# belinghy/SteppingStone

Measured on AMD Instinct MI355X. Metric: env-steps/sec (batched random-action rollout), higher is better.
Workload: dtype f32; 1 GPU; Walker3DStepperEnv-v0, 4096 envs per MI355X, curriculum 0 (flat terrain), on-device Philox U(-1,1) actions, auto-reset on; envs_total=4096, parallelism=env-shard x1, ranks=1, steps_per_launch=1000, prewarm_steps=256

## Files before the change

steppingstone_amd/csrc/ss_dynamics.hpp:

```cpp
#pragma once
#include "ss_math.hpp"
#include "ss_pair.hpp"

namespace ss {

constexpr float kH = 1.0f / 240.0f;
constexpr float kDt = 1.0f / 60.0f;
constexpr float kGrav = 9.8f;
constexpr float kPlankA = kStonePlankHalfLength, kPlankB = kStonePlankHalfWidth;
constexpr int kPgsIters = 5;
constexpr float kErp = 0.2f;
constexpr float kSlop = 0.001f;
constexpr float kVcorrMax = 2.0f;


constexpr int kWave = 64;
constexpr int kEnvsPerWave = 32;
constexpr int kLdsSlots = 40;
constexpr int kSlotsA = 20;
constexpr int kLdsC = 0;
constexpr int kLdsT = 18;
constexpr int kLdsHead = 36;
constexpr int kScalarBase = kSlotsA * kWave * 4;
constexpr int kRecWords = 9;
constexpr int kCholWords = 15 + 6;
constexpr int kHandJc = 0, kHandL0 = kHandJc + 8 * kRecWords, kHandLc = kHandL0 + kCholWords, kHandDet = 129, kHandAct = 146, kHandFloats = 158, kHandCs = kHandLc;
constexpr bool bias_offload(int helpers) { return helpers >= 3; }
constexpr bool spine_packed(int helpers) { return helpers >= 3; }
constexpr bool torques_paired(int helpers, bool kstep) { return helpers >= 3 && kstep; }
constexpr bool response_from_lds(int helpers, bool kstep) { return helpers >= 3 && kstep; }
constexpr int kHandBias = kHandJc;
static_assert(24 <= 3 * kRecWords, "biases fit the spine records' place");
constexpr int kHandRows = kHandJc + 3 * kRecWords;
constexpr int kHandRows3 = 160;
constexpr int kHandFloats3 = kHandRows3 + 40;
constexpr int kHandSlots3 = (kHandFloats3 + 3) / 4;
constexpr int hand_slots(int helpers) { return helpers >= 3 ? kHandSlots3 : (kHandFloats + 3) / 4; }
constexpr bool rows_offload(int helpers) { return helpers >= 3; }
constexpr int kHandSlots = (kHandFloats + 3) / 4;
static_assert(kLdsSlots + kHandSlots <= 80, "two helper-variant workgroups must fit the 160 KiB of a CU (16384 envs: 512 workgroups)");
static_assert(kHandRows + 40 <= kHandJc + 8 * kRecWords, "rows fit the leg records' place");
constexpr int kHandBase = kLdsSlots * kWave * 4;
constexpr int kFarWord0 = kHandLc;
constexpr int kFarBytes = (kHandBase + kFarWord0 * kWave) * 4;
static_assert(kFarBytes <= 65536, "every hand-off word beyond the offset field of the lane's own base goes through the far base");
constexpr bool hand_far(int idx) { return idx >= kFarWord0; }
constexpr int hand_far_offset(int idx) { return (idx - kFarWord0) * kWave * 4; }
constexpr int lds_bytes(int helpers) { return (kLdsSlots + hand_slots(helpers)) * kWave * 16; }
constexpr int hand_last_word(int helpers) { return hand_slots(helpers) * 4 - 1; }
static_assert(kHandFloats3 - 1 <= hand_last_word(3) && kHandFloats + 2 - 1 <= hand_last_word(1), "the words in use (one helper: + kHandOut2's two) are allocated");
static_assert(kFarBytes + (kWave - 1) * 4 + hand_far_offset(hand_last_word(1)) + 4 <= lds_bytes(1), "one helper: far base + largest word is inside the allocation");
static_assert(kFarBytes + (kWave - 1) * 4 + hand_far_offset(hand_last_word(3)) + 4 <= lds_bytes(3), "three helpers: far base + largest word is inside the allocation");
static_assert(hand_far_offset(kFarWord0) == 0 && hand_far_offset(hand_last_word(3)) < 65536 && hand_far_offset(hand_last_word(1)) < 65536,
              "every far offset fits the 16-bit offset field");
static_assert(hand_far_offset(1) - hand_far_offset(0) == 256 && hand_far_offset(hand_last_word(3)) / 256 <= 255,
              "far offsets are multiples of 256 B within ds_*2st64_b32's reach");
constexpr int NH = 12;
enum { S_ACT = 0, S_Q = 12, S_QD = 24, S_WLAM = 36, S_POS = 48, S_QUAT = 51, S_VW = 55, S_VV = 58, S_STP = 61, S_STN = 70,
       S_WKEY = 79, S_END = 80 };
static_assert(S_END <= (kLdsSlots - kSlotsA) * 4, "LDS scalar region overflow");
constexpr bool warm_in_lds(int helpers) { return helpers < 3; }

constexpr int kHalf[NH] = {0, 1, 2, 3, 4, 5, 6, 7, 13, 14, 15, 16};
constexpr int left_twin(int jr) { return jr < 3 ? jr : (jr < 8 ? jr + 5 : jr + 4); }
constexpr bool mirror_flips(int j) { return kAxis[j] != 1; }
__host__ __device__ constexpr float mirror_sign(int j, float m) { return mirror_flips(j) ? m : 1.f; }
__host__ __device__ constexpr float action_lane_sign(int jr, float m) {
  return jr < 3 ? mirror_sign(jr, m) : (float)kPolicySign[jr];
}
__host__ __device__ constexpr float policy_true_sign(int jr, int side) {
  return jr < 3 ? 1.f : (float)kPolicySign[jr] * ((mirror_flips(jr) && side) ? -1.f : 1.f);
}
constexpr int first_child_half(int b) {
  int r = -1;
  for (int i = 0; i < NH; ++i)
    if (kParent[kHalf[i]] == b) r = kHalf[i] + 1;
  return r;
}

#define SS_MEMBAR() asm volatile("" ::: "memory")
#if defined(__HIP_DEVICE_COMPILE__)
#define SS_WAVE_SYNC() asm volatile("" ::: "memory")
#else
#define SS_WAVE_SYNC() ss_host_wave_sync()
#endif

#if defined(SS_PROFILE_PHASES) && defined(__HIP_DEVICE_COMPILE__)
struct Prof { uint32_t t[16]; uint32_t last; };
#define SS_PROF_DECL Prof& prof,
#define SS_PROF_ARG prof,
#define SS_PROF_RAW(i) do { uint32_t _n = __builtin_amdgcn_readfirstlane((uint32_t)__builtin_amdgcn_s_memtime()); \
    prof.t[i] = __builtin_amdgcn_readfirstlane(prof.t[i] + (_n - __builtin_amdgcn_readfirstlane(prof.last))); prof.last = _n; } while (0)
#ifdef SS_PROFILE_EPILOGUE
#define SS_PROF(i) SS_PROF_RAW(0)
#define SS_PROFE(i) SS_PROF_RAW(i)
#else
#define SS_PROF(i) SS_PROF_RAW(i)
#define SS_PROFE(i) ((void)0)
#endif
#else
#define SS_PROFE(i) ((void)0)
struct Prof { int unused; };
#define SS_PROF_DECL
#define SS_PROF_ARG
#define SS_PROF(i) ((void)0)
#endif

#if defined(SS_FUZZ_SCHED) && defined(__HIP_DEVICE_COMPILE__)
__device__ __forceinline__ void ss_fuzz(uint32_t site) {
  uint32_t h = (uint32_t)__builtin_amdgcn_s_memtime() ^ (site * 0x9E3779B9u);
  h *= 0x85EBCA6Bu; h ^= h >> 13; h *= 0xC2B2AE35u; h ^= h >> 16;
  h = __builtin_amdgcn_readfirstlane(h);
  const uint32_t n = ((h >> 8) & 3u) == 0u ? (h & 255u) : (h & 15u);
#pragma unroll 1
  for (uint32_t i = 0; i < n; ++i) __builtin_amdgcn_s_sleep(1);
}
#define SS_FUZZ(site) ss_fuzz(site)
#else
#define SS_FUZZ(site) ((void)0)
#endif

constexpr bool cs_offload(int helpers) { return helpers >= 3; }

struct Lds {
  float* base;
  int lane;
  SSD float2& q2(int item) const { return reinterpret_cast<float2*>(base)[item * kWave + lane]; }
  SSD float& s(int idx) const { return base[kScalarBase + idx * kWave + lane]; }
  SSD float& hs(int idx) const {
#if defined(__HIP_DEVICE_COMPILE__)
    if (hand_far(idx)) {
      int off = kFarBytes + lane * 4;
      asm("" : "+v"(off));
      return *reinterpret_cast<float*>(reinterpret_cast<char*>(base) + off + hand_far_offset(idx));
    }
#endif
    return base[kHandBase + idx * kWave + lane];
  }
};

struct Stones {
  float p[3][3], nrm[3][3], tilt[3][2];
};

// ... 1290 lines not shown
```

steppingstone_amd/csrc/ss_kernels.hpp:

```cpp
#pragma once
#include <cstdlib>

#include "ss_dynamics.hpp"
#include "../../include/steppingstone.h"

namespace ss {

enum { F_POS = 0, F_QUAT = 3, F_VEL = 7, F_Q = 13, F_QD = 34, F_POT = 55, F_ZINIT = 56, F_EPRET = 57, F_NNDR = 58,
       F_STONE = 59, F_HEAD = 59 + 24, F_EPRET_LO = 59 + 30, NF = 59 + 30 + 1 };
enum { I_N = 0, I_COUNT = 1, I_ELAPSED = 2, I_RNG = 3, I_FLAGS = 4, I_PROV = 5, NI = 6 };
constexpr int kNumStones = 20;
constexpr int kNumSubsteps = 4;
constexpr float kDeg = 0.017453292519943295f;

struct Knobs {
  const float* prob;
  int per_env_prob;
  int curriculum;
  float power;
  int auto_reset;
};

struct Params {
  float* fstate;
// ... 201 lines not shown
  for (int i = 0; i < 3; ++i) { F[(F_VEL + i) * np] = s.v0.w[i]; F[(F_VEL + 3 + i) * np] = s.v0.v[i]; }
#pragma unroll
  for (int j = 0; j < NJ; ++j) { F[(F_Q + j) * np] = s.q[j]; F[(F_QD + j) * np] = s.qd[j]; }
}
SSD void load_cache(const Params& P, int e, Cache& c) {
  const float* F = P.fstate + e;
  const size_t np = (size_t)P.npad;
#pragma unroll
  for (int sl = 0; sl < 3; ++sl) {
#pragma unroll
    for (int i = 0; i < 3; ++i) { c.p[sl][i] = F[(F_STONE + sl * 8 + i) * np]; c.nrm[sl][i] = F[(F_STONE + sl * 8 + 3 + i) * np]; }
    c.tilt[sl][0] = F[(F_STONE + sl * 8 + 6) * np];
    c.tilt[sl][1] = F[(F_STONE + sl * 8 + 7) * np];
  }
}
SSD void store_cache(const Params& P, int e, const Cache& c) {
  float* F = P.fstate + e;
  const size_t np = (size_t)P.npad;
#pragma unroll
  for (int sl = 0; sl < 3; ++sl) {
#pragma unroll
    for (int i = 0; i < 3; ++i) { F[(F_STONE + sl * 8 + i) * np] = c.p[sl][i]; F[(F_STONE + sl * 8 + 3 + i) * np] = c.nrm[sl][i]; }
    F[(F_STONE + sl * 8 + 6) * np] = c.tilt[sl][0];
    F[(F_STONE + sl * 8 + 7) * np] = c.tilt[sl][1];
  }
}
SSD void store_headings(const Params& P, int e, const float (&h)[3][2]) {
  float* F = P.fstate + e;
  const size_t np = (size_t)P.npad;
#pragma unroll
  for (int sl = 0; sl < 3; ++sl) { F[(F_HEAD + sl * 2) * np] = h[sl][0]; F[(F_HEAD + sl * 2 + 1) * np] = h[sl][1]; }
}
SSD void cache_from_terrain(const Params& P, int e, int n, Cache& c, float (&hd)[3][2]) {
  const size_t np = (size_t)P.npad;
  const float* T = P.terrain + e;
  int idx[3] = {n - 1 < 0 ? 0 : n - 1, n, n + 1 > kNumStones - 1 ? kNumStones - 1 : n + 1};
#pragma unroll
  for (int sl = 0; sl < 3; ++sl) {
    int k = idx[sl];
#pragma unroll
    for (int i = 0; i < 3; ++i) c.p[sl][i] = T[(k * 6 + i) * np];
    float phi = T[(k * 6 + 3) * np], xt = T[(k * 6 + 4) * np], yt = T[(k * 6 + 5) * np];
    c.tilt[sl][0] = xt; c.tilt[sl][1] = yt;
    stone_normal(phi, xt, yt, c.nrm[sl]);
    sincosf(phi, &hd[sl][1], &hd[sl][0]);
  }
}

SSD void flat_path(Stones& c) {
#pragma unroll
  for (int sl = 0; sl < 3; ++sl) {
    c.p[sl][0] = 0.75f * (float)sl; c.p[sl][1] = 0.f; c.p[sl][2] = 0.f;
    c.nrm[sl][0] = 0.f; c.nrm[sl][1] = 0.f; c.nrm[sl][2] = 1.f;
    c.tilt[sl][0] = 0.f; c.tilt[sl][1] = 0.f;
  }
}
template <class Model, int GJ>
SSD float reset_angle(const uint32_t (&r)[6][4]) {
  constexpr float q0 = Model::q0[GJ], lo = Model::lo[GJ] + 0.02f, hi = Model::hi[GJ] - 0.02f;
  float q = q0 + 0.05f * (2.f * u01(r[GJ / 4][GJ % 4]) - 1.f);
  return fminf(fmaxf(q, lo), hi);
}

template <class Model>
SSD void env_reset(const Params& P, int e, Dyn& s, Cache& c, uint32_t& ctr, float& pot, float& z_init, float& nn_dr) {
  const size_t np = (size_t)P.npad;
  P.istate[e + I_PROV * np] = 0;
  flat_path(c);
  s.pos[0] = 0.f; s.pos[1] = 0.f; s.pos[2] = Model::stand_height + 0.01f;
  s.quat[0] = 1.f; s.quat[1] = s.quat[2] = s.quat[3] = 0.f;
#pragma unroll
  for (int i = 0; i < 3; ++i) { s.v0.w[i] = 0.f; s.v0.v[i] = 0.f; }
  uint32_t r[6][4];
#pragma unroll
  for (int b = 0; b < 6; ++b) env_block(P, e, ctr, r[b]);
  static_for<0, NJ>([&](auto Jc) {
    constexpr int j = decltype(Jc)::value;
    s.q[j] = reset_angle<Model, j>(r);
    s.qd[j] = 0.f;
  });
  z_init = s.pos[2];
  nn_dr = 0.75f;
  pot = -planar_dist(c.p[1], s.pos) / kDt;
}

constexpr int kMaxPeers = 8;
struct PeerTable {
  float* dst[kMaxPeers];
  uint32_t* flag[kMaxPeers];
  uint32_t* done_counter;
  int count;
  int rank;
  int n_local;
};

struct StepIO {
  const float* act;
  float* obs;
  float* rew;
  uint8_t* done;
  ss_info* info;
  uint64_t t;
  float* packed;
  int nsteps;
  const PeerTable* peers;
  uint32_t flag_value;
  long long packed_step_stride;
};

SSD void put_base(const Lds& L, float m, const float pos[3], const float quat[4], const float w[3], const float v[3]) {
  L.s(S_POS + 0) = pos[0]; L.s(S_POS + 1) = m * pos[1]; L.s(S_POS + 2) = pos[2];
  L.s(S_QUAT + 0) = quat[0]; L.s(S_QUAT + 1) = m * quat[1]; L.s(S_QUAT + 2) = quat[2]; L.s(S_QUAT + 3) = m * quat[3];
  L.s(S_VW + 0) = m * w[0]; L.s(S_VW + 1) = w[1]; L.s(S_VW + 2) = m * w[2];
  L.s(S_VV + 0) = v[0]; L.s(S_VV + 1) = m * v[1]; L.s(S_VV + 2) = v[2];
}
SSD void get_base(const Lds& L, float m, float pos[3], float quat[4], SV& v0) {
  pos[0] = L.s(S_POS); pos[1] = m * L.s(S_POS + 1); pos[2] = L.s(S_POS + 2);
  quat[0] = L.s(S_QUAT); quat[1] = m * L.s(S_QUAT + 1); quat[2] = L.s(S_QUAT + 2); quat[3] = m * L.s(S_QUAT + 3);
  v0 = SV{{m * L.s(S_VW), L.s(S_VW + 1), m * L.s(S_VW + 2)}, {L.s(S_VV), m * L.s(S_VV + 1), L.s(S_VV + 2)}};
}
SSD void put_joints(const Lds& L, float m, const float (&q)[NH], const float (&qd)[NH]) {
  static_for<0, NH>([&](auto Kc) {
    constexpr int k = decltype(Kc)::value, jr = kHalf[k];
    const float sg = mirror_sign(jr, m);
    L.s(S_Q + k) = sg * q[k];
    L.s(S_QD + k) = sg * qd[k];
  });
}
SSD void get_joints(const Lds& L, float m, float (&q)[NH], float (&qd)[NH]) {
  static_for<0, NH>([&](auto Kc) {
    constexpr int k = decltype(Kc)::value, jr = kHalf[k];
    const float sg = mirror_sign(jr, m);
    q[k] = sg * L.s(S_Q + k);
    qd[k] = sg * L.s(S_QD + k);
  });
}
SSD void put_stones(const Lds& L, float m, const Cache& c, const float (*h)[2] = nullptr) {
#pragma unroll
  for (int sl = 0; sl < 3; ++sl) {
    L.s(S_STP + sl * 3 + 0) = c.p[sl][0]; L.s(S_STP + sl * 3 + 1) = m * c.p[sl][1]; L.s(S_STP + sl * 3 + 2) = c.p[sl][2];
    L.s(S_STN + sl * 3 + 0) = c.nrm[sl][0]; L.s(S_STN + sl * 3 + 1) = m * c.nrm[sl][1]; L.s(S_STN + sl * 3 + 2) = c.nrm[sl][2];
    if (h) L.q2(kLdsHead + sl) = make_float2(h[sl][0], m * h[sl][1]);
  }
}
SSD void load_actions(const float* act_row, int side, float (&ain)[NH]) {
  static_for<0, NH>([&](auto Kc) {
    constexpr int k = decltype(Kc)::value, jr = kHalf[k];
    constexpr int jl = left_twin(jr);
    ain[k] = act_row[side ? jl : jr];
  });
}
SSD void put_actions(const Lds& L, float m, const float (&ain)[NH]) {
  static_for<0, NH>([&](auto Kc) {
    constexpr int k = decltype(Kc)::value, jr = kHalf[k];
    const float sg = action_lane_sign(jr, m);
    const float x = ain[k];
    float a = fminf(fmaxf(x, -1.f), 1.f);
    a = (x != x) ? x : a;
    L.s(S_ACT + k) = sg * a;
  });
}

template <bool ACT>
SSD void load_in(const Params& P, int e, const float* act_row, int side, float m, const Lds& L, float (&ain)[NH]) {
  const size_t np = (size_t)P.npad;
  const float* F = P.fstate + e;
// ... 104 lines not shown
      if (io.done) io.done[e] = o.d ? 1 : 0;
      if (packed_layout) {
        stage[SS_OBS_DIM] = o.r;
        stage[SS_OBS_DIM + 1] = o.d ? 1.f : 0.f;
      }
      istage[0] = SS_F2U(o.inf.ep_ret); istage[1] = SS_F2U(o.inf.ep_len);
      istage[2] = (uint32_t)o.inf.bad_transition; istage[3] = (uint32_t)o.inf.steps_reached; istage[4] = (uint32_t)o.inf.update_terrain;
      istage[5] = SS_F2U(o.inf.ep_ret_lo);
#pragma unroll
      for (int i = 0; i < 3; ++i) Fo[(F_POS + i) * np] = o.pos[i];
#pragma unroll
      for (int i = 0; i < 4; ++i) Fo[(F_QUAT + i) * np] = o.quat[i];
#pragma unroll
      for (int i = 0; i < 3; ++i) { Fo[(F_VEL + i) * np] = o.v0.w[i]; Fo[(F_VEL + 3 + i) * np] = o.v0.v[i]; }
    }
  }
  {
    SS_WAVE_SYNC();
    const int env0 = (lane_global - lane) >> 1;
    const int nleft = P.n - env0;
    const int nvalid = nleft <= 0 ? 0 : (kEnvsPerWave < nleft ? kEnvsPerWave : nleft);
    auto copy_block = [&](float* dst, int nfl) {
      if ((reinterpret_cast<uintptr_t>(dst) & 15u) == 0) {
        const int n4 = nfl >> 2;
        float4* d4 = reinterpret_cast<float4*>(dst);
        const float4* s4 = reinterpret_cast<const float4*>(lds);
#pragma unroll 1
        for (int g = lane; g < n4; g += kWave) copy_out(&d4[g], s4[g]);
        for (int g = (n4 << 2) + lane; g < nfl; g += kWave) copy_out(&dst[g], lds[g]);
      } else {
#pragma unroll 1
        for (int g = lane; g < nfl; g += kWave) copy_out(&dst[g], lds[g]);
      }
    };
    if (io.obs) {
      float* og = io.obs + (size_t)env0 * SS_OBS_DIM;
      if (!packed_layout) {
        copy_block(og, nvalid * SS_OBS_DIM);
      } else {
#pragma unroll 1
        for (int g = lane; g < nvalid * SS_OBS_DIM; g += kWave) {
          const int el = g / SS_OBS_DIM, idx = g - el * SS_OBS_DIM;
          copy_out(&og[g], lds[el * kPackW + idx]);
        }
      }
    }
    if (io.packed) {
      float* pk = io.packed + (size_t)env0 * kPackW;
      if constexpr (ROLLOUT) pk += (long long)kstep * io.packed_step_stride;
      copy_block(pk, nvalid * kPackW);
    }
    if (io.info) {
      uint32_t* ig = reinterpret_cast<uint32_t*>(io.info + env0);
      const uint32_t* is = reinterpret_cast<const uint32_t*>(lds) + kInfoBase;
      for (int g = lane; g < nvalid * SS_INFO_WORDS; g += kWave) copy_out(&ig[g], is[g]);
    }
#if defined(__HIP_DEVICE_COMPILE__)
    if constexpr (!ROLLOUT) {
      if (io.peers) {
        constexpr int kPack = SS_OBS_DIM + 2;
        const PeerTable* T = io.peers;
        const int G = T->count;
        const size_t row0 = (size_t)T->rank * (size_t)T->n_local + (size_t)env0;
#pragma unroll 1
        for (int p = 0; p < G; ++p) copy_block(T->dst[p] + row0 * kPack, nvalid * kPack);
        __threadfence_system();
        if (lane == 0) {
          const uint32_t prev = atomicAdd(T->done_counter, 1u);
          if ((prev + 1u) % gridDim.x == 0u) {
            __threadfence_system();
            for (int p = 0; p < G; ++p)
              __hip_atomic_store(T->flag[p] + T->rank, io.flag_value, __ATOMIC_RELEASE, __HIP_MEMORY_SCOPE_SYSTEM);
          }
        }
      }
    }
#endif
  }
}

constexpr bool out_offload(int helpers, bool rollout) { return rollout && helpers >= 3; }
constexpr int kHandOut = kHandDet, kHandOut2 = kHandFloats;
static_assert(kHandOut2 + 2 <= kHandSlots * 4, "hand-off region");
#if !defined(SS_HOST_HARNESS)
template <class Model, bool ROLLOUT>
__device__ __forceinline__ void emit_from_handoff(const Params& P, const StepIO& io, const Lds& L, int lane, int lane_global, int kstep,
                                                  float* lds) {
  const int e_raw = lane_global >> 1, side = lane_global & 1;
  const bool valid = e_raw < P.n;
  const int e = valid ? e_raw : P.n - 1;
  const float m = side ? -1.f : 1.f;
  StepOut o;
  get_base(L, m, o.pos, o.quat, o.v0);
  get_joints(L, m, o.qt, o.qdt);
  o.r = L.hs(kHandOut + 0);
  o.z_init = L.hs(kHandOut + 1);
  {
    const float w = L.hs(kHandOut + 2), w2 = xchg(w);
    o.inf.ep_ret = side ? w2 : w;
    o.inf.ep_ret_lo = side ? w : w2;
  }
  const int bits = __builtin_bit_cast(int, L.hs(kHandOut2 + 0));
  o.d = bits & 1;
  o.inf.bad_transition = (bits >> 1) & 1;
  o.inf.update_terrain = (bits >> 2) & 1;
  o.do_reset = (bits >> 3) & 1;
  o.flags = (bits >> 4) & 3;
  o.inf.steps_reached = (bits >> 8) & 31;
  o.inf.ep_len = (float)((bits >> 16) & 0xffff);
#pragma unroll
  for (int i = 0; i < 5; ++i) { o.tgt[0][i] = L.hs(kHandOut + 3 + i); o.tgt[1][i] = L.hs(kHandOut + 8 + i); }
  quat_roll_pitch_cs(o.quat, o.roll, o.pitch, o.cyaw, o.syaw);
  emit_outputs<Model, ROLLOUT>(P, io, o, e, side, valid, lane, lane_global, kstep, lds);
}
#endif

template <class Write>
SSD void random_actions_half(const Params& P, int e, int side, float m, uint32_t tt, Write&& write) {
  uint32_t ra[6][4];
#pragma unroll
  for (int b = 0; b < 6; ++b) philox4x32_10(6u * tt + b, 1u, P.env_offset + ((uint32_t)e & P.id_mask), 0u, P.seed_lo, P.seed_hi, ra[b]);
  static_for<0, NH>([&](auto Kc) {
    constexpr int k = decltype(Kc)::value, jr = kHalf[k];
    constexpr int jl = left_twin(jr);
    const float sg = action_lane_sign(jr, m);
    const uint32_t bits = side ? ra[jl / 4][jl % 4] : ra[jr / 4][jr % 4];
    write(k, sg * (2.f * u01(bits) - 1.f));
  });
}

struct StepScore {
  float pot_prev;
  bool d;
  int bad;
  float r, roll, pitch, cyaw, syaw;
};
SSD StepScore step_score(SS_PROF_DECL const float (&pos)[3], const float (&quat)[4], const Cache& c, const float (&target_old)[3],
                         const float (&sole)[2][3], float pot_prev, int advanced, int n, int elapsed, bool finite, float step_bonus,
                         float e_sum, float a2, int at_limit) {
  StepScore o;
  float pot = -planar_dist(target_old, pos) / kDt;
  SS_PROFE(4);
  float progress = pot - pot_prev;
  o.pot_prev = advanced ? -planar_dist(c.p[1], pos) / kDt : pot;
  float target_bonus = (n == kNumStones - 1 && planar_dist(c.p[1], pos) < 0.15f) ? 2.f : 0.f;
  float zs = fminf(sole[0][2], sole[1][2]);
  float tall_bonus = (pos[2] - zs > 0.7f) ? 2.f : -1.f;
  float zlow = fminf(fminf(c.p[0][2], c.p[1][2]), c.p[2][2]);
  bool d = (tall_bonus < 0.f) || (pos[2] < zlow + 0.3f) || !finite;
  bool timeout = elapsed >= SS_MAX_EPISODE_STEPS;
  o.bad = timeout ? 1 : 0;
  o.d = d || timeout;
  quat_roll_pitch_cs(quat, o.roll, o.pitch, o.cyaw, o.syaw);
  float posture = 0.f;
  if (!(o.pitch > -0.2f && o.pitch < 0.4f)) posture += fabsf(o.pitch);
  if (!(o.roll > -0.4f && o.roll < 0.4f)) posture += fabsf(o.roll);
  float energy = (4.5f / NJ) * (e_sum / NJ) + (0.225f / NJ) * (a2 / NJ);
  float r = progress + step_bonus + target_bonus + tall_bonus - energy - posture - 0.1f * (float)at_limit;
  if (!finite || !finite_bits(r)) r = 0.f;
  o.r = r;
  SS_PROFE(5);
  return o;
}
SSD void ep_return_add(float& ep_ret, float& ep_lo, float r) {
  const float s = ep_ret + r, bb = s - ep_ret;
  const float err = (ep_ret - (s - bb)) + (r - bb);
// ... 21 lines not shown
  const float my_sole[3] = {fr.sole[0], m * fr.sole[1], fr.sole[2]};
  float ot_sole[3];
#pragma unroll
  for (int i = 0; i < 3; ++i) ot_sole[i] = xchg(my_sole[i]);
  const int ot_contact = xchg_i(fr.contact), ot_target = xchg_i(fr.on_target);
  float sole[2][3];
#pragma unroll
  for (int i = 0; i < 3; ++i) { sole[0][i] = side ? ot_sole[i] : my_sole[i]; sole[1][i] = side ? my_sole[i] : ot_sole[i]; }
  o.flags = side ? (ot_contact | (fr.contact << 1)) : (fr.contact | (ot_contact << 1));
  const int on_target = fr.on_target | ot_target;
  SS_PROFE(2);
  float accv = 0.f, e_sum = 0.f, a2 = 0.f;
  int at_limit = 0;
  static_for<0, NH>([&](auto Kc) {
    constexpr int k = decltype(Kc)::value, jr = kHalf[k];
    constexpr float mid = 0.5f * (Model::lo[jr] + Model::hi[jr]);
    constexpr float span = Model::hi[jr] - Model::lo[jr];
    const float q = L.s(S_Q + k), qd = L.s(S_QD + k), a = L.s(S_ACT + k);
    const bool mine = (jr >= 3) || (side == 0);
    accv += q + qd;
    if (mine) {
      e_sum += fabsf(a * (0.1f * qd));
      a2 += a * a;
      if (fabsf(2.f * (q - mid) / span) > 0.99f) at_limit += 1;
    }
  });
  accv += pos[0] + pos[1] + pos[2] + quat[0] + quat[1] + quat[2] + quat[3];
#pragma unroll
  for (int i = 0; i < 3; ++i) accv += v0.w[i] + v0.v[i];
  e_sum += xchg(e_sum);
  a2 += xchg(a2);
  at_limit += xchg_i(at_limit);
  const bool finite = finite_bits(accv) && (xchg_i(finite_bits(accv) ? 1 : 0) != 0);
  SS_PROFE(3);

  float target_old[3] = {c.p[1][0], c.p[1][1], c.p[1][2]};
  float step_bonus = 0.f;
  int advanced = 0;
#pragma unroll
  for (int sl = 0; sl < 3; ++sl) { hd[sl][0] = 1.f; hd[sl][1] = 0.f; }
  if (on_target != 0) {
    count += 1;
    if (count == 1) {
      float d0 = planar_dist(sole[0], target_old), d1 = planar_dist(sole[1], target_old);
      step_bonus = 50.f * expf(-fminf(d0, d1) / 0.25f);
    }
    if (count >= 2 && n < kNumStones - 1) {
      n += 1;
      count = 0;
      advanced = 1;
#pragma unroll
      for (int i = 0; i < 3; ++i) {
        c.p[0][i] = c.p[1][i]; c.nrm[0][i] = c.nrm[1][i];
        c.p[1][i] = c.p[2][i]; c.nrm[1][i] = c.nrm[2][i];
      }
      c.tilt[0][0] = c.tilt[1][0]; c.tilt[0][1] = c.tilt[1][1];
      c.tilt[1][0] = c.tilt[2][0]; c.tilt[1][1] = c.tilt[2][1];
      const float2 h1 = L.q2(kLdsHead + 1), h2 = L.q2(kLdsHead + 2);
      hd[0][0] = h1.x; hd[0][1] = m * h1.y;
      hd[1][0] = h2.x; hd[1][1] = m * h2.y;
      hd[2][0] = h2.x; hd[2][1] = m * h2.y;
      if (n + 1 <= kNumStones - 1) nn_dr = draw(ctr, n + 1, c.p[2], c.nrm[2], c.tilt[2], hd[2], store);
      L.q2(kLdsHead + 0) = h1;
      L.q2(kLdsHead + 1) = h2;
      L.q2(kLdsHead + 2) = make_float2(hd[2][0], m * hd[2][1]);
    }
  }
  o.advanced = advanced;
  const StepScore sc = step_score(SS_PROF_ARG pos, quat, c, target_old, sole, pot_prev, advanced, n, elapsed, finite, step_bonus, e_sum, a2, at_limit);
  pot_prev = sc.pot_prev;
  o.d = sc.d; o.bad = sc.bad; o.r = sc.r; o.roll = sc.roll; o.pitch = sc.pitch; o.cyaw = sc.cyaw; o.syaw = sc.syaw;
  ep_return_add(ep_ret, ep_lo, sc.r);
}

template <class Model, bool RANDOM_ACT, int HELPERS = 0, bool ROLLOUT = false>
SSD void step_env(const Params& P, const StepIO& io, int lane_global, int lane, float* lds) {
  static_assert(!ROLLOUT || RANDOM_ACT, "a multi-step launch draws its actions on the device");
  constexpr bool kOffload =
#if defined(__HIP_DEVICE_COMPILE__)
      out_offload(HELPERS, ROLLOUT);
#else
      false;
#endif
  const int e_raw = lane_global >> 1, side = lane_global & 1;
  const bool valid = e_raw < P.n;
  int e = valid ? e_raw : P.n - 1;
  const size_t np = (size_t)P.npad;
  const float m = side ? -1.f : 1.f;
  const Lds L{lds, lane};
  float ain[NH];
  load_in<!RANDOM_ACT>(P, e, RANDOM_ACT ? nullptr : io.act + (size_t)e * NJ, side, m, L, ain);

  const int nsteps = ROLLOUT ? io.nsteps : 1;
#pragma unroll 1
  for (int kstep = 0; kstep < nsteps; ++kstep) {
  SS_FUZZ(0x60u);
  if constexpr (RANDOM_ACT) {
    bool drawn = false;
    if constexpr (ROLLOUT && HELPERS > 1) {
      if (kstep > 0) {
        float a[NH];
#pragma unroll
        for (int k = 0; k < NH; ++k) a[k] = L.hs(kHandAct + k);
#pragma unroll
        for (int k = 0; k < NH; ++k) L.s(S_ACT + k) = a[k];
        drawn = true;
      }
    }
    if (!drawn) random_actions_half(P, e, side, m, (uint32_t)io.t + (uint32_t)kstep, [&](int k, float a) { L.s(S_ACT + k) = a; });
  } else {
    put_actions(L, m, ain);
  }

  const float power = P.knobs->power;
  FootReport fr;
#if defined(SS_PROFILE_PHASES) && defined(__HIP_DEVICE_COMPILE__)
  Prof prof;
#pragma unroll
  for (int i = 0; i < 16; ++i) prof.t[i] = 0;
  prof.last = (uint32_t)__builtin_amdgcn_s_memtime();
#endif
  Warm wm;
  warm_clear(wm);
  if constexpr (warm_in_lds(HELPERS)) L.s(S_WKEY) = 0.f;
#pragma unroll 1
  for (int k = 0; k < kNumSubsteps; ++k) substep<Model, HELPERS, ROLLOUT>(SS_PROF_ARG power, fr, L, wm);
  SS_FUZZ(0x61u);
  SS_PROF(12);
  SS_MEMBAR();
  SS_OPAQUE(e);
  const float* F = P.fstate + e;
  const Knobs K = *P.knobs;
  Cache c;
  load_cache(P, e, c);
  float pot_prev = F[F_POT * np], z_init = F[F_ZINIT * np];
  float ep_ret = F[F_EPRET * np], ep_lo = F[F_EPRET_LO * np], nn_dr = F[F_NNDR * np];
  int n = P.istate[e + I_N * np], count = P.istate[e + I_COUNT * np], elapsed = P.istate[e + I_ELAPSED * np];
  uint32_t ctr = (uint32_t)P.istate[e + I_RNG * np];
  SS_PROFE(1);

  float pos[3], quat[4];
  SV v0;
  get_base(L, m, pos, quat, v0);
  elapsed += 1;
  const float my_sole[3] = {fr.sole[0], m * fr.sole[1], fr.sole[2]};
  float ot_sole[3];
#pragma unroll
  for (int i = 0; i < 3; ++i) ot_sole[i] = xchg(my_sole[i]);
  const int ot_contact = xchg_i(fr.contact), ot_target = xchg_i(fr.on_target);
  float sole[2][3];
#pragma unroll
  for (int i = 0; i < 3; ++i) { sole[0][i] = side ? ot_sole[i] : my_sole[i]; sole[1][i] = side ? my_sole[i] : ot_sole[i]; }
  int flags = side ? (ot_contact | (fr.contact << 1)) : (fr.contact | (ot_contact << 1));
  const int on_target = fr.on_target | ot_target;
  SS_PROFE(2);
  float accv = 0.f, e_sum = 0.f, a2 = 0.f;
  int at_limit = 0;
  static_for<0, NH>([&](auto Kc) {
    constexpr int k = decltype(Kc)::value, jr = kHalf[k];
    constexpr float mid = 0.5f * (Model::lo[jr] + Model::hi[jr]);
    constexpr float span = Model::hi[jr] - Model::lo[jr];
    const float q = L.s(S_Q + k), qd = L.s(S_QD + k), a = L.s(S_ACT + k);
    const bool mine = (jr >= 3) || (side == 0);
    accv += q + qd;
    if (mine) {
      e_sum += fabsf(a * (0.1f * qd));
      a2 += a * a;
      if (fabsf(2.f * (q - mid) / span) > 0.99f) at_limit += 1;
    }
  });
  accv += pos[0] + pos[1] + pos[2] + quat[0] + quat[1] + quat[2] + quat[3];
#pragma unroll
  for (int i = 0; i < 3; ++i) accv += v0.w[i] + v0.v[i];
  e_sum += xchg(e_sum);
  a2 += xchg(a2);
  at_limit += xchg_i(at_limit);
  const bool finite = finite_bits(accv) && (xchg_i(finite_bits(accv) ? 1 : 0) != 0);
  SS_PROFE(3);

  float target_old[3] = {c.p[1][0], c.p[1][1], c.p[1][2]};
  float step_bonus = 0.f;
  int advanced = 0;
  float hd[3][2] = {{1.f, 0.f}, {1.f, 0.f}, {1.f, 0.f}};
  if (on_target != 0) {
    count += 1;
    if (count == 1) {
      float d0 = planar_dist(sole[0], target_old), d1 = planar_dist(sole[1], target_old);
      step_bonus = 50.f * expf(-fminf(d0, d1) / 0.25f);
    }
    if (count >= 2 && n < kNumStones - 1) {
      n += 1;
      count = 0;
      advanced = 1;
#pragma unroll
      for (int i = 0; i < 3; ++i) {
        c.p[0][i] = c.p[1][i]; c.nrm[0][i] = c.nrm[1][i];
        c.p[1][i] = c.p[2][i]; c.nrm[1][i] = c.nrm[2][i];
      }
      c.tilt[0][0] = c.tilt[1][0]; c.tilt[0][1] = c.tilt[1][1];
      c.tilt[1][0] = c.tilt[2][0]; c.tilt[1][1] = c.tilt[2][1];
      const float2 h1 = L.q2(kLdsHead + 1), h2 = L.q2(kLdsHead + 2);
      hd[0][0] = h1.x; hd[0][1] = m * h1.y;
      hd[1][0] = h2.x; hd[1][1] = m * h2.y;
      hd[2][0] = h2.x; hd[2][1] = m * h2.y;
      if (n + 1 <= kNumStones - 1) nn_dr = draw_stone(P, K, e, ctr, n + 1, c.p[2], c.nrm[2], c.tilt[2], hd[2], valid && side == 0);
      L.q2(kLdsHead + 0) = h1;
      L.q2(kLdsHead + 1) = h2;
      L.q2(kLdsHead + 2) = make_float2(hd[2][0], m * hd[2][1]);
    }
  }
  const StepScore sc = step_score(SS_PROF_ARG pos, quat, c, target_old, sole, pot_prev, advanced, n, elapsed, finite, step_bonus, e_sum, a2, at_limit);
  pot_prev = sc.pot_prev;
  const bool d = sc.d;
  const int bad = sc.bad;
  const float r = sc.r, roll = sc.roll, pitch = sc.pitch, cyaw = sc.cyaw, syaw = sc.syaw;
  ep_return_add(ep_ret, ep_lo, r);
  ss_info inf;
  inf.ep_ret = ep_ret;
  inf.ep_ret_lo = ep_lo;
  inf.ep_len = (float)elapsed;
  inf.bad_transition = bad;
  inf.steps_reached = n;
  inf.update_terrain = advanced;
  const bool do_reset = d && K.auto_reset;
  SS_PROFE(6);
  uint32_t rr[6][4];
  if (do_reset) {
    if (valid && side == 0) P.istate[e + I_PROV * np] = 0;
    flat_path(c);
#pragma unroll
    for (int sl = 0; sl < 3; ++sl) {
      hd[sl][0] = 1.f; hd[sl][1] = 0.f;
      L.q2(kLdsHead + sl) = make_float2(1.f, 0.f);
    }
    pos[0] = 0.f; pos[1] = 0.f; pos[2] = Model::stand_height + 0.01f;
    quat[0] = 1.f; quat[1] = quat[2] = quat[3] = 0.f;
#pragma unroll
    for (int i = 0; i < 3; ++i) { v0.w[i] = 0.f; v0.v[i] = 0.f; }
    {
      uint32_t c3 = ctr + (side ? 3u : 0u), mine[3][4];
#pragma unroll
      for (int b = 0; b < 3; ++b) env_block(P, e, c3, mine[b]);
#pragma unroll
      for (int b = 0; b < 3; ++b)
#pragma unroll
        for (int i = 0; i < 4; ++i) {
          const uint32_t other = xchg_u32(mine[b][i]);
          rr[b][i] = side ? other : mine[b][i];
          rr[3 + b][i] = side ? mine[b][i] : other;
        }
      ctr += 6u;
    }
    z_init = pos[2];
    nn_dr = 0.75f;
    pot_prev = -planar_dist(c.p[1], pos) / kDt;
    n = 1; count = 0; elapsed = 0; flags = 0; ep_ret = 0.f; ep_lo = 0.f;
  }
  SS_PROFE(7);
  float qt[NH], qdt[NH];
  static_for<0, NH>([&](auto Kc) {
    constexpr int k = decltype(Kc)::value, jr = kHalf[k];
    constexpr int jl = left_twin(jr);
    const float sg = mirror_sign(jr, m);
    if (do_reset) {
      qt[k] = side ? reset_angle<Model, jl>(rr) : reset_angle<Model, jr>(rr);
      qdt[k] = 0.f;
    } else {
      qt[k] = sg * L.s(S_Q + k);
      qdt[k] = sg * L.s(S_QD + k);
    }
  });
  SS_PROFE(8);
  SS_FUZZ(0x62u);
  if constexpr (ROLLOUT) {
    if (do_reset) {
      put_base(L, m, pos, quat, v0.w, v0.v);
      put_joints(L, m, qt, qdt);
    }
    if (advanced || do_reset) put_stones(L, m, c);
  }
  if constexpr (kOffload) {
    L.hs(kHandOut + 0) = r;
    L.hs(kHandOut + 1) = z_init;
    L.hs(kHandOut + 2) = side ? inf.ep_ret_lo : inf.ep_ret;
    const int bits = (d ? 1 : 0) | (inf.bad_transition << 1) | (inf.update_terrain << 2) | ((do_reset ? 1 : 0) << 3) | (flags << 4) |
                     (inf.steps_reached << 8) | ((int)inf.ep_len << 16);
    L.hs(kHandOut2 + 0) = __builtin_bit_cast(float, bits);
#pragma unroll
    for (int i = 0; i < 3; ++i) { L.hs(kHandOut + 3 + i) = c.p[1][i]; L.hs(kHandOut + 8 + i) = c.p[2][i]; }
#pragma unroll
    for (int i = 0; i < 2; ++i) { L.hs(kHandOut + 6 + i) = c.tilt[1][i]; L.hs(kHandOut + 11 + i) = c.tilt[2][i]; }
  } else {
    StepOut o;
#pragma unroll
    for (int i = 0; i < 3; ++i) o.pos[i] = pos[i];
#pragma unroll
    for (int i = 0; i < 4; ++i) o.quat[i] = quat[i];
    o.v0 = v0;
#pragma unroll
    for (int k = 0; k < NH; ++k) { o.qt[k] = qt[k]; o.qdt[k] = qdt[k]; }
    o.r = r; o.z_init = z_init; o.roll = roll; o.pitch = pitch; o.cyaw = cyaw; o.syaw = syaw;
    o.d = d ? 1 : 0; o.flags = flags; o.do_reset = do_reset ? 1 : 0;
#pragma unroll
    for (int i = 0; i < 3; ++i) { o.tgt[0][i] = c.p[1][i]; o.tgt[1][i] = c.p[2][i]; }
#pragma unroll
    for (int i = 0; i < 2; ++i) { o.tgt[0][3 + i] = c.tilt[1][i]; o.tgt[1][3 + i] = c.tilt[2][i]; }
    o.inf = inf;
    emit_outputs<Model, ROLLOUT>(P, io, o, e, side, valid, lane, lane_global, kstep, lds);
  }
  if (valid && side == 0) {
  SS_PROFE(9);
    float* Fo = P.fstate + e;
    if (advanced || do_reset) {
      store_cache(P, e, c);
      store_headings(P, e, hd);
    }
    Fo[F_POT * np] = pot_prev;
    Fo[F_ZINIT * np] = z_init;
    Fo[F_EPRET * np] = ep_ret;
    Fo[F_EPRET_LO * np] = ep_lo;
    Fo[F_NNDR * np] = nn_dr;
    P.istate[e + I_N * np] = n;
    P.istate[e + I_COUNT * np] = count;
    P.istate[e + I_ELAPSED * np] = elapsed;
    P.istate[e + I_RNG * np] = (int)ctr;
    P.istate[e + I_FLAGS * np] = flags;
  }
  SS_MEMBAR();
#if defined(SS_PROFILE_PHASES) && defined(__HIP_DEVICE_COMPILE__)
  SS_PROFE(10);
  SS_PROF(13);
  if (lane == 0 && P.prof)
    for (int i = 0; i < 16; ++i) atomicAdd(P.prof + i, (unsigned long long)prof.t[i]);
#endif
  }
#if defined(__HIP_DEVICE_COMPILE__)
  if constexpr (out_offload(HELPERS, ROLLOUT)) __syncthreads();
#endif
}

#ifndef SS_HOST_HARNESS
template <class Model, bool RANDOM_ACT>
__global__ __launch_bounds__(kWave, 1) void step_kernel(Params P, StepIO io) {
  __shared__ float4 lds4[kLdsSlots * kWave];
  step_env<Model, RANDOM_ACT>(P, io, blockIdx.x * kWave + threadIdx.x, threadIdx.x, reinterpret_cast<float*>(lds4));
}
template <class Model, bool RANDOM_ACT, int HELPERS>
__global__ __launch_bounds__(kWave * (1 + HELPERS), 1) void step_kernel_helped(Params P, StepIO io) {
  __shared__ float4 lds4[(kLdsSlots + hand_slots(HELPERS)) * kWave];
  const int wave = __builtin_amdgcn_readfirstlane(threadIdx.x >> 6), lane = threadIdx.x & (kWave - 1);
  float* lds = reinterpret_cast<float*>(lds4);
  SS_FUZZ(0x70u + wave);
  if (wave == 0) {
    step_env<Model, RANDOM_ACT, HELPERS>(P, io, blockIdx.x * kWave + lane, lane, lds);
  } else {
    const Lds L{lds, lane};
#pragma unroll 1
    for (int k = 0; k < kNumSubsteps; ++k) helper_substep<Model, HELPERS, 6>(wave - 1, L, [](int) {});
  }
}
template <class Model>
__global__ __launch_bounds__(kWave, 1) void rollout_kernel(Params P, StepIO io) {
  __shared__ float4 lds4[kLdsSlots * kWave];
  step_env<Model, true, 0, true>(P, io, blockIdx.x * kWave + threadIdx.x, threadIdx.x, reinterpret_cast<float*>(lds4));
}
template <class Model, int HELPERS>
__global__ __launch_bounds__(kWave * (1 + HELPERS), 1) void rollout_kernel_helped(Params P, StepIO io) {
  __shared__ float4 lds4[(kLdsSlots + hand_slots(HELPERS)) * kWave];
  const int wave = __builtin_amdgcn_readfirstlane(threadIdx.x >> 6), lane = threadIdx.x & (kWave - 1);
  float* lds = reinterpret_cast<float*>(lds4);
  SS_FUZZ(0x70u + wave);
  if (wave == 0) {
    step_env<Model, true, HELPERS, true>(P, io, blockIdx.x * kWave + lane, lane, lds);
  } else {
    const Lds L{lds, lane};
    const int lane_global = blockIdx.x * kWave + lane, side = lane_global & 1;
    const int e = min(lane_global >> 1, P.n - 1);
    const float m = side ? -1.f : 1.f;
#pragma unroll 1
    for (int kstep = 0; kstep < io.nsteps; ++kstep)
#pragma unroll 1
      for (int k = 0; k < kNumSubsteps; ++k)
        helper_substep<Model, HELPERS, 4>(wave - 1, L, [&](int helper) {
          if (k != 0) return;
          SS_FUZZ(0x80u + helper);
          constexpr int kActHelper = 1, kEmitHelper = HELPERS - 1;
          if (HELPERS > 1 && helper == kActHelper && kstep + 1 < io.nsteps)
            random_actions_half(P, e, side, m, (uint32_t)io.t + (uint32_t)kstep + 1u, [&](int j, float a) { L.hs(kHandAct + j) = a; });
          if (out_offload(HELPERS, true) && helper == kEmitHelper && kstep > 0) emit_from_handoff<Model, true>(P, io, L, lane, lane_global, kstep - 1, lds);
        });
    if constexpr (out_offload(HELPERS, true)) {
      __syncthreads();
      SS_FUZZ(0x90u + wave);
      if (wave == 2) emit_from_handoff<Model, true>(P, io, L, lane, lane_global, io.nsteps - 1, lds);
    }
  }
}

template <class Model>
SSD void reset_env(const Params& P, int e, float* obs_row) {
  const size_t np = (size_t)P.npad;
  Dyn s;
  Cache c;
  uint32_t ctr = (uint32_t)P.istate[e + I_RNG * np];
  float pot, z_init, nn_dr;
  env_reset<Model>(P, e, s, c, ctr, pot, z_init, nn_dr);
  store_dyn(P, e, s);
  store_cache(P, e, c);
  const float straight[3][2] = {{1.f, 0.f}, {1.f, 0.f}, {1.f, 0.f}};
  store_headings(P, e, straight);
  P.fstate[e + F_POT * np] = pot;
  P.fstate[e + F_ZINIT * np] = z_init;
  P.fstate[e + F_EPRET * np] = 0.f;
  P.fstate[e + F_EPRET_LO * np] = 0.f;
  P.fstate[e + F_NNDR * np] = nn_dr;
  P.istate[e + I_N * np] = 1;
  P.istate[e + I_COUNT * np] = 0;
  P.istate[e + I_ELAPSED * np] = 0;
  P.istate[e + I_RNG * np] = (int)ctr;
  P.istate[e + I_FLAGS * np] = 0;
  if (obs_row) {
    float o[SS_OBS_DIM];
    write_obs<Model>(s, z_init, 0, c, o);
#pragma unroll
    for (int i = 0; i < SS_OBS_DIM; ++i) obs_row[i] = o[i];
  }
}

template <class Model>
__global__ __launch_bounds__(kWave) void reset_kernel(Params P, float* obs) {
  const int e = blockIdx.x * kWave + threadIdx.x;
  if (e >= P.n) return;
  reset_env<Model>(P, e, obs ? obs + (size_t)e * SS_OBS_DIM : nullptr);
}

template <class Model>
__global__ __launch_bounds__(kWave) void obs_kernel(Params P, float* obs) {
  const int e = blockIdx.x * kWave + threadIdx.x;
  if (e >= P.n) return;
  const size_t np = (size_t)P.npad;
  Dyn s;
  Cache c;
  load_dyn(P, e, s);
  load_cache(P, e, c);
  float o[SS_OBS_DIM];
  write_obs<Model>(s, P.fstate[e + F_ZINIT * np], P.istate[e + I_FLAGS * np], c, o);
#pragma unroll
  for (int i = 0; i < SS_OBS_DIM; ++i) obs[(size_t)e * SS_OBS_DIM + i] = o[i];
}
#endif

SSD void pack_env(const Params& P, int e, float* packed, size_t row) {
  const size_t np = (size_t)P.npad;
  float* o = packed + row * SS_STATE_DIM;
  for (int i = 0; i < 59; ++i) o[i] = P.fstate[e + (size_t)i * np];
  o[59] = (float)P.istate[e + I_N * np];
  o[60] = (float)P.istate[e + I_COUNT * np];
  o[61] = (float)P.istate[e + I_ELAPSED * np];
  uint32_t ctr = (uint32_t)P.istate[e + I_RNG * np];
  o[62] = (float)(ctr & 0xFFFFu);
  o[63] = (float)(ctr >> 16);
  o[64] = (float)P.istate[e + I_FLAGS * np];
  const int prov = P.istate[e + I_PROV * np];
  for (int i = 0; i < 120; ++i) {
    const int k = i / 6;
    o[65 + i] = k < prov ? P.terrain[e + (size_t)i * np] : (i % 6 == 0 ? 0.75f * (float)k : 0.f);
  }
  o[185] = P.fstate[e + (size_t)F_EPRET_LO * np];
}
SSD void pack_env(const Params& P, int e, float* packed) { pack_env(P, e, packed, (size_t)e); }
SSD void unpack_env(const Params& P, int e, const float* packed, size_t row) {
  const size_t np = (size_t)P.npad;
  const float* o = packed + row * SS_STATE_DIM;
// ... 20 lines not shown
```

Measured before the change: 97.94 million env-steps/s.

## Precompute reset joint pose on a helper wave and hand it off via LDS

When three or more helper waves are present, a helper wave precomputes the Philox-based reset joint angles for the current RNG counter and stores them in the LDS words the warm-start impulses would otherwise use. On reset, the main wave copies the pose from LDS and skips its own RNG and angle computation. The main wave publishes its counter through a hand-off word so the helper can recompute when it changes. If the counter moved within the same step, the main wave falls back to computing the pose itself. This takes reset work off the critical main wave, at the cost of extra helper work, LDS traffic and more synchronisation complexity.

Result: faster. 99.48 million env-steps/s (median of 6 runs) (+1.6%).

```diff
diff --git a/steppingstone_amd/csrc/ss_dynamics.hpp b/steppingstone_amd/csrc/ss_dynamics.hpp
--- a/steppingstone_amd/csrc/ss_dynamics.hpp
+++ b/steppingstone_amd/csrc/ss_dynamics.hpp
@@ -60,6 +60,12 @@
        S_WKEY = 79, S_END = 80 };
 static_assert(S_END <= (kLdsSlots - kSlotsA) * 4, "LDS scalar region overflow");
 constexpr bool warm_in_lds(int helpers) { return helpers < 3; }
+constexpr bool reset_pose_offload(int helpers, bool kstep) { return helpers >= 3 && kstep; }
+constexpr int S_POSE = S_WLAM;
+static_assert(!(reset_pose_offload(0, true) && warm_in_lds(0)) && !(reset_pose_offload(1, true) && warm_in_lds(1)) &&
+              !(reset_pose_offload(2, true) && warm_in_lds(2)) && !(reset_pose_offload(3, true) && warm_in_lds(3)),
+              "the reset pose lives where the warm-start impulses would: only a kernel that keeps those in registers has the words to spare");
+static_assert(S_POSE + NH <= S_POS, "twelve words");
 
 constexpr int kHalf[NH] = {0, 1, 2, 3, 4, 5, 6, 7, 13, 14, 15, 16};
 constexpr int left_twin(int jr) { return jr < 3 ? jr : (jr < 8 ? jr + 5 : jr + 4); }
diff --git a/steppingstone_amd/csrc/ss_kernels.hpp b/steppingstone_amd/csrc/ss_kernels.hpp
--- a/steppingstone_amd/csrc/ss_kernels.hpp
+++ b/steppingstone_amd/csrc/ss_kernels.hpp
@@ -307,6 +307,26 @@
   z_init = s.pos[2];
   nn_dr = 0.75f;
   pot = -planar_dist(c.p[1], s.pos) / kDt;
+}
+template <class Model, class Write>
+SSD void reset_pose_half(const Params& P, int e, int side, float m, uint32_t ctr, Write&& write) {
+  uint32_t rr[6][4], c3 = ctr + (side ? 3u : 0u), mine[3][4];
+#pragma unroll
+  for (int b = 0; b < 3; ++b) env_block(P, e, c3, mine[b]);
+#pragma unroll
+  for (int b = 0; b < 3; ++b)
+#pragma unroll
+    for (int i = 0; i < 4; ++i) {
+      const uint32_t other = xchg_u32(mine[b][i]);
+      rr[b][i] = side ? other : mine[b][i];
+      rr[3 + b][i] = side ? mine[b][i] : other;
+    }
+  static_for<0, NH>([&](auto Kc) {
+    constexpr int k = decltype(Kc)::value, jr = kHalf[k];
+    constexpr int jl = left_twin(jr);
+    const float qt = side ? reset_angle<Model, jl>(rr) : reset_angle<Model, jr>(rr);
+    write(k, mirror_sign(jr, m) * qt);
+  });
 }
 
 constexpr int kMaxPeers = 8;
@@ -577,6 +597,8 @@
 constexpr bool out_offload(int helpers, bool rollout) { return rollout && helpers >= 3; }
 constexpr int kHandOut = kHandDet, kHandOut2 = kHandFloats;
 static_assert(kHandOut2 + 2 <= kHandSlots * 4, "hand-off region");
+constexpr int kHandCtr = kHandOut2 + 1;
+static_assert(kHandCtr < kHandRows3, "below the rows' own words");
 #if !defined(SS_HOST_HARNESS)
 template <class Model, bool ROLLOUT>
 __device__ __forceinline__ void emit_from_handoff(const Params& P, const StepIO& io, const Lds& L, int lane, int lane_global, int kstep,
@@ -764,6 +786,13 @@
 #else
       false;
 #endif
+  constexpr bool kPose =
+#if defined(__HIP_DEVICE_COMPILE__)
+      reset_pose_offload(HELPERS, ROLLOUT);
+#else
+      false;
+#endif
+  static_assert(!kPose || kOffload, "the pose's helper and the counter's hand-off word are the output stage's kernel's");
   const int e_raw = lane_global >> 1, side = lane_global & 1;
   const bool valid = e_raw < P.n;
   int e = valid ? e_raw : P.n - 1;
@@ -819,6 +848,7 @@
   float ep_ret = F[F_EPRET * np], ep_lo = F[F_EPRET_LO * np], nn_dr = F[F_NNDR * np];
   int n = P.istate[e + I_N * np], count = P.istate[e + I_COUNT * np], elapsed = P.istate[e + I_ELAPSED * np];
   uint32_t ctr = (uint32_t)P.istate[e + I_RNG * np];
+  const uint32_t ctr_in = ctr;
   SS_PROFE(1);
 
   float pos[3], quat[4];
@@ -907,6 +937,7 @@
   const bool do_reset = d && K.auto_reset;
   SS_PROFE(6);
   uint32_t rr[6][4];
+  const bool pose_stale = kPose && do_reset && ctr != ctr_in;
   if (do_reset) {
     if (valid && side == 0) P.istate[e + I_PROV * np] = 0;
     flat_path(c);
@@ -919,7 +950,9 @@
     quat[0] = 1.f; quat[1] = quat[2] = quat[3] = 0.f;
 #pragma unroll
     for (int i = 0; i < 3; ++i) { v0.w[i] = 0.f; v0.v[i] = 0.f; }
-    {
+    if constexpr (kPose) {
+      ctr += 6u;
+    } else {
       uint32_t c3 = ctr + (side ? 3u : 0u), mine[3][4];
 #pragma unroll
       for (int b = 0; b < 3; ++b) env_block(P, e, c3, mine[b]);
@@ -940,25 +973,46 @@
   }
   SS_PROFE(7);
   float qt[NH], qdt[NH];
-  static_for<0, NH>([&](auto Kc) {
-    constexpr int k = decltype(Kc)::value, jr = kHalf[k];
-    constexpr int jl = left_twin(jr);
-    const float sg = mirror_sign(jr, m);
-    if (do_reset) {
-      qt[k] = side ? reset_angle<Model, jl>(rr) : reset_angle<Model, jr>(rr);
-      qdt[k] = 0.f;
-    } else {
-      qt[k] = sg * L.s(S_Q + k);
-      qdt[k] = sg * L.s(S_QD + k);
-    }
-  });
+  if constexpr (!kPose) {
+    static_for<0, NH>([&](auto Kc) {
+      constexpr int k = decltype(Kc)::value, jr = kHalf[k];
+      constexpr int jl = left_twin(jr);
+      const float sg = mirror_sign(jr, m);
+      if (do_reset) {
+        qt[k] = side ? reset_angle<Model, jl>(rr) : reset_angle<Model, jr>(rr);
+        qdt[k] = 0.f;
+      } else {
+        qt[k] = sg * L.s(S_Q + k);
+        qdt[k] = sg * L.s(S_QD + k);
+      }
+    });
+  }
   SS_PROFE(8);
   SS_FUZZ(0x62u);
   if constexpr (ROLLOUT) {
     if (do_reset) {
       put_base(L, m, pos, quat, v0.w, v0.v);
-      put_joints(L, m, qt, qdt);
-    }
+      if constexpr (kPose) {
+        float qp[NH];
+#pragma unroll
+        for (int k = 0; k < NH; ++k) qp[k] = L.s(S_POSE + k);
+        const float zm = __builtin_bit_cast(float, side ? 0x80000000u : 0u);
+        static_for<0, NH>([&](auto Kc) {
+          constexpr int k = decltype(Kc)::value;
+          L.s(S_Q + k) = qp[k];
+          L.s(S_QD + k) = mirror_flips(kHalf[k]) ? zm : 0.f;
+        });
+      } else {
+        put_joints(L, m, qt, qdt);
+      }
+    }
+#if defined(__HIP_DEVICE_COMPILE__)
+    if constexpr (kPose) {
+      if (__any(pose_stale)) {
+        if (pose_stale) reset_pose_half<Model>(P, e, side, m, ctr - 6u, [&](int k, float q) { L.s(S_Q + k) = q; });
+      }
+    }
+#endif
     if (advanced || do_reset) put_stones(L, m, c);
   }
   if constexpr (kOffload) {
@@ -968,6 +1022,7 @@
     const int bits = (d ? 1 : 0) | (inf.bad_transition << 1) | (inf.update_terrain << 2) | ((do_reset ? 1 : 0) << 3) | (flags << 4) |
                      (inf.steps_reached << 8) | ((int)inf.ep_len << 16);
     L.hs(kHandOut2 + 0) = __builtin_bit_cast(float, bits);
+    if constexpr (kPose) L.hs(kHandCtr) = __builtin_bit_cast(float, ctr);
 #pragma unroll
     for (int i = 0; i < 3; ++i) { L.hs(kHandOut + 3 + i) = c.p[1][i]; L.hs(kHandOut + 8 + i) = c.p[2][i]; }
 #pragma unroll
@@ -1059,10 +1114,14 @@
     const int lane_global = blockIdx.x * kWave + lane, side = lane_global & 1;
     const int e = min(lane_global >> 1, P.n - 1);
     const float m = side ? -1.f : 1.f;
+    constexpr int kPoseHelper = 0;
+    uint32_t ctr_pose = 0u;
+    if constexpr (reset_pose_offload(HELPERS, true))
+      if (wave - 1 == kPoseHelper) ctr_pose = (uint32_t)P.istate[e + I_RNG * (size_t)P.npad];
 #pragma unroll 1
     for (int kstep = 0; kstep < io.nsteps; ++kstep)
 #pragma unroll 1
-      for (int k = 0; k < kNumSubsteps; ++k)
+      for (int k = 0; k < kNumSubsteps; ++k) {
         helper_substep<Model, HELPERS, 4>(wave - 1, L, [&](int helper) {
           if (k != 0) return;
           SS_FUZZ(0x80u + helper);
@@ -1071,6 +1130,17 @@
             random_actions_half(P, e, side, m, (uint32_t)io.t + (uint32_t)kstep + 1u, [&](int j, float a) { L.hs(kHandAct + j) = a; });
           if (out_offload(HELPERS, true) && helper == kEmitHelper && kstep > 0) emit_from_handoff<Model, true>(P, io, L, lane, lane_global, kstep - 1, lds);
         });
+        if constexpr (reset_pose_offload(HELPERS, true)) {
+          if (k == 0 && wave - 1 == kPoseHelper) {
+            SS_FUZZ(0xA0u);
+            const uint32_t ctr_now = kstep == 0 ? ctr_pose : __builtin_bit_cast(uint32_t, L.hs(kHandCtr));
+            if (kstep == 0 || __any(ctr_now != ctr_pose)) {
+              ctr_pose = ctr_now;
+              reset_pose_half<Model>(P, e, side, m, ctr_now, [&](int j, float q) { L.s(S_POSE + j) = q; });
+            }
+          }
+        }
+      }
     if constexpr (out_offload(HELPERS, true)) {
       __syncthreads();
       SS_FUZZ(0x90u + wave);
```
